# facebookresearch/Active-3D-Vision-and-Touch

Measured on AMD Instinct MI355X. Metric: mesh-recon iters/sec (fwd+bwd, 2562-vert GCN + 10k-pt Chamfer) at bs=64, higher is better.
Workload: dtype f32; 1 GPU; icosphere-4 template (2562 verts, 5120 faces), 3-stage GCN 20x300 cut 0.33, bs=64/GPU, 10000-pt Chamfer x3 draws, Adam, ellipsoid clouds (BASELINE.json configs[1]); global_batch=64, parallelism=dp1

## Files before the change

active-3d-vision-and-touch_amd/csrc/capi.hip:

```cpp
#include <stdarg.h>
#include <stdlib.h>
#include <string.h>

#include "../../include/a3vt.h"
#include <atomic>
#include <mutex>
#include <unordered_map>

#include "common.h"
#include "kernels.h"

namespace a3vt {

static thread_local char g_err[512] = "";

void set_error(const char *fmt, ...) {
  va_list ap;
  va_start(ap, fmt);
  vsnprintf(g_err, sizeof(g_err), fmt, ap);
  va_end(ap);
}

__device__ float g_zero_page[64];
static const float *zero_page() {
// ... 1634 lines not shown
  return launch_conv5_up3(grad_out, batch, out_height, out_width, image, grad_in, static_cast<hipStream_t>(stream));
}

size_t a3vt_conv5_wrw_scratch_bytes(int cin, int cout) {
  return ((cin == 16 || cin == 32) && (cout == 16 || cout == 32)) || (cin == 3 && (cout == 3 || cout == 16)) ? conv5_wrw_scratch_bytes(cin, cout) : 0;
}

int a3vt_conv5_weight_grad(const void *x, const void *grad_out, int batch, int height, int width, int cin, int cout, int stride,
                           float *grad_weight, void *scratch, size_t scratch_bytes, void *stream) {
  A3VT_CHECK_ARG(x && grad_out && grad_weight && scratch);
  A3VT_CHECK_ARG(conv5_shape_ok(cin, cout, stride));
  A3VT_CHECK_ARG(batch > 0 && height >= 3 && width >= 3 && (long long)batch * height * width <= (1ll << 31) / 32);
  A3VT_CHECK_ARG((reinterpret_cast<uintptr_t>(scratch) & 15) == 0);
  A3VT_CHECK_ARG((reinterpret_cast<uintptr_t>(x) & (cin == 3 ? 1 : 15)) == 0 && (reinterpret_cast<uintptr_t>(grad_out) & (cout == 3 ? 1 : 15)) == 0);
  A3VT_CHECK_ARG(scratch_bytes >= conv5_wrw_scratch_bytes(cin, cout));
  ProfScope psc(PROF_ENC, static_cast<hipStream_t>(stream));
  return launch_conv5_wrw(x, grad_out, batch, height, width, cin, cout, stride, grad_weight, scratch, static_cast<hipStream_t>(stream));
}

int a3vt_adam_chunk_elems(void) { return adam_chunk_elems(); }

int a3vt_adam_step(void *const *param, const void *const *grad, void *const *exp_avg, void *const *exp_avg_sq,
                   const long long *numel, const int *chunk_tensor, const long long *chunk_off, int n_chunks, double lr, double beta1,
                   double beta2, double eps, double weight_decay, long long step, void *stream) {
  A3VT_CHECK_ARG(n_chunks >= 0 && step >= 1);
  A3VT_CHECK_ARG(n_chunks == 0 || (param && grad && exp_avg && exp_avg_sq && numel && chunk_tensor && chunk_off));
  A3VT_CHECK_ARG(lr >= 0.0 && beta1 >= 0.0 && beta1 < 1.0 && beta2 >= 0.0 && beta2 < 1.0 && eps >= 0.0 && weight_decay >= 0.0);
  ProfScope psc(PROF_OPT, static_cast<hipStream_t>(stream));
  return launch_adam(param, grad, exp_avg, exp_avg_sq, numel, chunk_tensor, chunk_off, n_chunks, lr, beta1, beta2, eps, weight_decay, step,
                     static_cast<hipStream_t>(stream));
}

int a3vt_adam_step_clamp(void *const *param, void *const *grad, void *const *exp_avg, void *const *exp_avg_sq, const long long *numel,
                         const int *chunk_tensor, const long long *chunk_off, int n_chunks, double lr, double beta1, double beta2,
                         double eps, double weight_decay, long long step, double grad_clamp, void *stream) {
  A3VT_CHECK_ARG(n_chunks >= 0 && step >= 1 && grad_clamp > 0.0);
  A3VT_CHECK_ARG(n_chunks == 0 || (param && grad && exp_avg && exp_avg_sq && numel && chunk_tensor && chunk_off));
  A3VT_CHECK_ARG(lr >= 0.0 && beta1 >= 0.0 && beta1 < 1.0 && beta2 >= 0.0 && beta2 < 1.0 && eps >= 0.0 && weight_decay >= 0.0);
  ProfScope psc(PROF_OPT, static_cast<hipStream_t>(stream));
  return launch_adam(param, const_cast<const void *const *>(grad), exp_avg, exp_avg_sq, numel, chunk_tensor, chunk_off, n_chunks, lr, beta1,
                     beta2, eps, weight_decay, step, static_cast<hipStream_t>(stream), grad_clamp);
}

int a3vt_profile_enable(int on) {
  g_prof.on = on != 0;
  g_prof.used = 0;
  return 0;
}

int a3vt_profile_read_classes(double *total_ms, int *count, int n) {
  A3VT_CHECK_ARG(total_ms && count && n >= 0);
  for (int c = 0; c < n; ++c) { total_ms[c] = 0.0; count[c] = 0; }
  for (int i = 0; i < g_prof.used; ++i) {
    if (hipEventSynchronize(g_prof.ev[i][1]) != hipSuccess) { set_error("profile_read: event sync failed"); return -2; }
    float ms = 0.f;
    if (hipEventElapsedTime(&ms, g_prof.ev[i][0], g_prof.ev[i][1]) != hipSuccess) continue;
    if (g_prof.cls[i] >= n) continue;
    total_ms[g_prof.cls[i]] += ms;
    count[g_prof.cls[i]] += 1;
  }
  g_prof.used = 0;
  return PROF_CLASSES;
}

int a3vt_profile_read(double *total_ms, int *count) {
  const int rc = a3vt_profile_read_classes(total_ms, count, 3);
  return rc < 0 ? rc : 0;
}

int a3vt_dbg_path_counts(long long *counts, int n, int reset) {
  A3VT_CHECK_ARG(n >= 0 && (counts != nullptr || n == 0));
  for (int i = 0; i < n; ++i) counts[i] = i < PATH_COUNT ? g_path_counts[i].load(std::memory_order_relaxed) : 0;
  if (reset)
    for (auto &c : g_path_counts) c.store(0, std::memory_order_relaxed);
  return PATH_COUNT;
}

int a3vt_dbg_csr_algo(int algo) {
  A3VT_CHECK_ARG(algo >= 0 && algo <= 2);
  g_csr_algo = algo;
  return 0;
}

int a3vt_split3_bf16(const float *x, size_t n, uint16_t *hi, uint16_t *mid, uint16_t *lo, void *stream) {
  A3VT_CHECK_ARG(n == 0 || (x && hi && mid && lo));
  return launch_split3(x, n, hi, mid, lo, static_cast<hipStream_t>(stream));
}

int a3vt_check_finite(const float *data, size_t n, int32_t *flag, void *stream) {
  A3VT_CHECK_ARG(data && flag);
  return launch_check_finite(data, n, flag, static_cast<hipStream_t>(stream));
}

}
```

active-3d-vision-and-touch_amd/csrc/gcn_csrq.hip:

```cpp
#include "common.h"
#include "kernels.h"

namespace a3vt {

using f32x4 = __attribute__((ext_vector_type(4))) float;

constexpr int kCsrqThreads = 512;
constexpr int kHeavyDegQ = 64;
constexpr int kEllW = 8;

using i32x2 = __attribute__((ext_vector_type(2))) int;
__device__ __forceinline__ float bits_to_f32(int x) { return __builtin_bit_cast(float, x); }
__device__ __forceinline__ int f32_to_bits(float x) { return __builtin_bit_cast(int, x); }
__global__ void csr_ell_build_kernel(const int32_t *__restrict__ rowptr, const int32_t *__restrict__ colidx,
                                     const float *__restrict__ val, int n_vert, i32x2 *__restrict__ ell,
                                     int32_t *__restrict__ degs) {
  const int v = blockIdx.x * blockDim.x + threadIdx.x;
  if (v >= n_vert) return;
  const int e0 = rowptr[v], n = rowptr[v + 1] - e0;
  degs[v] = n;
#pragma unroll
  for (int j = 0; j < kEllW; ++j)
    ell[(size_t)j * n_vert + v] = j < n ? i32x2{colidx[e0 + j], f32_to_bits(val[e0 + j])} : i32x2{n_vert, 0};
}
size_t csrq_ell_ints(int n_vert) { return (size_t)n_vert * (2 * kEllW + 1) + 64; }
int launch_csrq_ell(const int32_t *rowptr, const int32_t *col, const float *val, int n_vert, int32_t *ell, hipStream_t s) {
  A3VT_LAUNCH(csr_ell_build_kernel, dim3(cdiv(n_vert, 256)), dim3(256), 0, s, rowptr, col, val, n_vert,
              reinterpret_cast<i32x2 *>(ell), ell + (size_t)n_vert * 2 * kEllW);
  A3VT_CHECK_LAUNCH();
  return 0;
}

template <int MODE, int VPT>
__global__ __launch_bounds__(kCsrqThreads) void csrq_kernel(const float *__restrict__ srcq, int nq, int parts,
                                                            const float *__restrict__ bias, int c,
                                                            const int32_t *__restrict__ rowptr,
                                                            const int32_t *__restrict__ colidx,
                                                            const float *__restrict__ val, int n_vert, int batch,
                                                            float *__restrict__ dst, int nq_dst,
                                                            uint8_t *__restrict__ signq, int relu, int heavy_thresh,
                                                            float *__restrict__ db_slab,
                                                            const int32_t *__restrict__ ellbuf) {
  extern __shared__ __attribute__((aligned(16))) float lds_raw[];
  __shared__ float red[2][kCsrqThreads / 64][4];
  const i32x2 *ell = reinterpret_cast<const i32x2 *>(ellbuf);
  const int32_t *degs = ellbuf + (size_t)n_vert * 2 * kEllW;
  f32x4 *tile0 = reinterpret_cast<f32x4 *>(lds_raw);
  const int xcd = blockIdx.x & 7, loc = blockIdx.x >> 3;
  const int jm = loc / parts, part = loc - jm * parts;
  const int b = xcd + 8 * jm;
  if (b >= batch) return;
  const int q_lo = part * nq / parts, q_hi = (part + 1) * nq / parts;
  if (q_lo >= q_hi) return;

  int vv[VPT], dg[VPT];
  bool on[VPT];
  int cj[VPT][kEllW];
  float wj[VPT][kEllW];
#pragma unroll
  for (int k = 0; k < VPT; ++k) {
    const int v = threadIdx.x + k * kCsrqThreads;
    on[k] = v < n_vert;
    vv[k] = on[k] ? v : n_vert - 1;
    dg[k] = degs[vv[k]];
#pragma unroll
    for (int j = 0; j < kEllW; ++j) {
      const i32x2 e = ell[(size_t)j * n_vert + vv[k]];
      const int e0 = e[0], e1 = e[1];
      cj[k][j] = e0;
      wj[k][j] = bits_to_f32(e1);
    }
  }

  auto fetch = [&](int q, int k, f32x4 &v4, unsigned &bits) {
    const size_t plane = ((size_t)b * nq + q) * n_vert;
    v4 = reinterpret_cast<const f32x4 *>(srcq)[plane + vv[k]];
    bits = MODE == 1 ? signq[plane + vv[k]] : 0u;
  };
  auto park = [&](f32x4 *tile, int q, int k, f32x4 v4, unsigned bits) {
    if (MODE == 1) {
#pragma unroll
      for (int t = 0; t < 4; ++t) v4[t] = ((bits >> t) & 1u) ? v4[t] : 0.f;
    }
    (void)q;
    tile[vv[k]] = v4;
  };

  if (threadIdx.x < 2) tile0[(size_t)threadIdx.x * (n_vert + 1) + n_vert] = f32x4{0.f, 0.f, 0.f, 0.f};
  {
    f32x4 v4[VPT];
    unsigned bits[VPT];
#pragma unroll
    for (int k = 0; k < VPT; ++k) fetch(q_lo, k, v4[k], bits[k]);
#pragma unroll
    for (int k = 0; k < VPT; ++k) park(tile0, q_lo, k, v4[k], bits[k]);
  }
  __syncthreads();

  for (int q = q_lo; q < q_hi; ++q) {
    const int par = (q - q_lo) & 1;
    const f32x4 *tile = tile0 + (size_t)par * (n_vert + 1);
    f32x4 *tnext = tile0 + (size_t)(par ^ 1) * (n_vert + 1);
    const int ch = q * 4;
    const size_t plane = ((size_t)b * nq + q) * n_vert;
    const int qn = q + 1 < q_hi ? q + 1 : q;
    f32x4 nv4[VPT];
    unsigned nbits[VPT];
#pragma unroll
    for (int k = 0; k < VPT; ++k) fetch(qn, k, nv4[k], nbits[k]);
    f32x4 bs = {0.f, 0.f, 0.f, 0.f};
    if (MODE == 0) {
#pragma unroll
      for (int t = 0; t < 4; ++t)
        if (ch + t < c) bs[t] = bias[ch + t];
    }
    f32x4 bsum = {0.f, 0.f, 0.f, 0.f};
#pragma unroll
    for (int k = 0; k < VPT; ++k) {
      __builtin_amdgcn_sched_barrier(0);
      const int v = vv[k];
      const f32x4 own = tile[v];
      if (MODE == 1) {
#pragma unroll
        for (int t = 0; t < 4; ++t) bsum[t] += on[k] ? own[t] : 0.f;
      }
      f32x4 acc = {0.f, 0.f, 0.f, 0.f};
#pragma unroll
      for (int j = 0; j < kEllW; ++j) {
        {
          const f32x4 r = tile[cj[k][j]];
          const float w = wj[k][j];
          acc[0] = __builtin_fmaf(w, r[0], acc[0]);
          acc[1] = __builtin_fmaf(w, r[1], acc[1]);
          acc[2] = __builtin_fmaf(w, r[2], acc[2]);
          acc[3] = __builtin_fmaf(w, r[3], acc[3]);
        }
      }
      if (dg[k] > kEllW && dg[k] <= heavy_thresh) {
        const int ea = rowptr[v];
        for (int e = ea + kEllW; e < ea + dg[k]; ++e) {
          const f32x4 r = tile[colidx[e]];
          const float w = val[e];
#pragma unroll
          for (int t = 0; t < 4; ++t) acc[t] = __builtin_fmaf(w, r[t], acc[t]);
        }
      }
      if (!on[k] || dg[k] > heavy_thresh) continue;
      f32x4 o;
      if (MODE == 0) {
        unsigned bits = 0;
#pragma unroll
        for (int t = 0; t < 4; ++t) {
          const float pre = ch + t < c ? acc[t] + bs[t] : own[t];
          o[t] = (pre > 0.f || !relu) ? pre : 0.f;
          bits |= (pre > 0.f ? 1u : 0u) << t;
        }
        if (signq) signq[plane + v] = (uint8_t)bits;
      } else {
#pragma unroll
        for (int t = 0; t < 4; ++t) o[t] = ch + t < c ? acc[t] : own[t];
      }
      *reinterpret_cast<f32x4 *>(dst + ((((size_t)b * nq_dst + q) * n_vert) + v) * 4) = o;
    }
    __builtin_amdgcn_sched_barrier(0);
    if (MODE == 1) {
#pragma unroll
      for (int t = 0; t < 4; ++t) bsum[t] = wave_sum(bsum[t]);
      if ((threadIdx.x & 63) == 0) {
#pragma unroll
        for (int t = 0; t < 4; ++t) red[par][threadIdx.x >> 6][t] = bsum[t];
      }
    }
    if (q + 1 < q_hi) {
#pragma unroll
      for (int k = 0; k < VPT; ++k) park(tnext, q + 1, k, nv4[k], nbits[k]);
    }
    __syncthreads();
    if (MODE == 1 && threadIdx.x < 4) {
      float sacc = 0.f;
#pragma unroll
      for (int w = 0; w < kCsrqThreads / 64; ++w) sacc += red[par][w][threadIdx.x];
      db_slab[(size_t)b * (nq * 4) + ch + threadIdx.x] = sacc;
    }
  }
}

template <int MODE>
__global__ __launch_bounds__(256) void csrq_heavy_kernel(const float *__restrict__ srcq, int nq,
                                                         const float *__restrict__ bias, int c,
                                                         const int32_t *__restrict__ rowptr,
                                                         const int32_t *__restrict__ colidx,
                                                         const float *__restrict__ val, int n_vert, int batch,
                                                         const int32_t *__restrict__ heavy, float *__restrict__ dst,
                                                         int nq_dst, uint8_t *__restrict__ signq, int relu) {
  __shared__ f32x4 red[8][32];
  const int hl = threadIdx.x & 31, sub = threadIdx.x >> 5;
  const int count = heavy[0];
  const bool on = hl < nq;
  const int ch = hl * 4;
  for (long long item = blockIdx.x; item < (long long)count * batch; item += gridDim.x) {
    const int v = heavy[64 + (int)(item % count)];
    const long long b = item / count;
    const size_t plane = ((size_t)b * nq + (on ? hl : 0)) * n_vert;
    const f32x4 *src = reinterpret_cast<const f32x4 *>(srcq) + plane;
    const int e0 = rowptr[v], e1 = rowptr[v + 1];
    const int per = ((e1 - e0 + 7) / 8 + 3) & ~3;
    const int s0 = min(e1, e0 + sub * per), s1 = min(e1, s0 + per);
    f32x4 acc = {0.f, 0.f, 0.f, 0.f};
    if (on) {
      for (int e = s0; e < s1; ++e) {
        const int cc = colidx[e];
        f32x4 r = src[cc];
        if (MODE == 1) {
          const unsigned bits = signq[plane + cc];
#pragma unroll
          for (int t = 0; t < 4; ++t) r[t] = ((bits >> t) & 1u) ? r[t] : 0.f;
        }
#pragma unroll
        for (int t = 0; t < 4; ++t) acc[t] = __builtin_fmaf(val[e], r[t], acc[t]);
      }
    }
    red[sub][hl] = acc;
    __syncthreads();
    if (sub == 0 && on) {
      f32x4 a = red[0][hl];
#pragma unroll
      for (int r = 1; r < 8; ++r) a += red[r][hl];
      f32x4 own = src[v];
      f32x4 o;
      if (MODE == 0) {
        unsigned bits = 0;
#pragma unroll
        for (int t = 0; t < 4; ++t) {
          const float pre = ch + t < c ? a[t] + bias[ch + t] : own[t];
          o[t] = (pre > 0.f || !relu) ? pre : 0.f;
          bits |= (pre > 0.f ? 1u : 0u) << t;
        }
        if (signq) signq[plane + v] = (uint8_t)bits;
      } else {
        const unsigned bits = signq[plane + v];
#pragma unroll
        for (int t = 0; t < 4; ++t) {
          own[t] = ((bits >> t) & 1u) ? own[t] : 0.f;
          o[t] = ch + t < c ? a[t] : own[t];
        }
      }
      *reinterpret_cast<f32x4 *>(dst + ((((size_t)b * nq_dst + hl) * n_vert) + v) * 4) = o;
    }
    __syncthreads();
  }
}

int csrq_max_degree() { return kEllW; }
bool csrq_fits(int n_vert, int cut_len) {
  return cut_len > 0 && pad4(cut_len) <= 128 && n_vert <= 6 * kCsrqThreads && ((size_t)n_vert + 1) * 32 <= 158 * 1024;
}

template <int MODE, int VPT>
static int launch_csrq_vpt(const float *srcq, int nq, const float *bias, int c, const int32_t *rowptr, const int32_t *col,
                           const float *val, const int32_t *heavy, const int32_t *ell, int n_vert, int batch, float *dst,
                           int nq_dst, uint8_t *signq, int relu, float *db_slab, hipStream_t s) {
  const size_t shmem = ((size_t)n_vert + 1) * 32;
  static OncePerDevice once;
  once.run([] {
    (void)hipFuncSetAttribute((const void *)csrq_kernel<MODE, VPT>, hipFuncAttributeMaxDynamicSharedMemorySize, 158 * 1024);
  });
  int parts = 256 / (((batch + 7) / 8) * 8);
  parts = parts < 1 ? 1 : parts > nq ? nq : parts;
  const int grid = 8 * ((batch + 7) / 8) * parts;
  A3VT_LAUNCH((csrq_kernel<MODE, VPT>), dim3(grid), dim3(kCsrqThreads), shmem, s, srcq, nq, parts, bias, c, rowptr, col, val,
              n_vert, batch, dst, nq_dst, signq, relu, heavy ? kHeavyDegQ : 0x7fffffff, db_slab, ell);
  A3VT_CHECK_LAUNCH();
  return 0;
}

template <int MODE>
static int launch_csrq(const float *srcq, const float *bias, int c, const int32_t *rowptr, const int32_t *col,
                       const float *val, const int32_t *heavy, const int32_t *ell, int n_vert, int batch, float *dst,
                       int nq_dst, uint8_t *signq, int relu, float *db_slab, hipStream_t s) {
  const int nq = pad4(c) / 4;
  if (!csrq_fits(n_vert, c) || nq_dst < nq || (MODE == 1 && (!signq || !db_slab))) {
    set_error("csrq: n_vert=%d c=%d output planes=%d unsupported", n_vert, c, nq_dst);
    return -1;
  }
  int rc;
  if (n_vert <= 4 * kCsrqThreads)
    rc = launch_csrq_vpt<MODE, 4>(srcq, nq, bias, c, rowptr, col, val, heavy, ell, n_vert, batch, dst, nq_dst, signq, relu, db_slab, s);
  else
    rc = launch_csrq_vpt<MODE, 6>(srcq, nq, bias, c, rowptr, col, val, heavy, ell, n_vert, batch, dst, nq_dst, signq, relu, db_slab, s);
  if (rc) return rc;
  if (heavy) {
    A3VT_LAUNCH(csrq_heavy_kernel<MODE>, dim3(2048), dim3(256), 0, s, srcq, nq, bias, c, rowptr, col, val, n_vert, batch,
                heavy, dst, nq_dst, signq, relu);
    A3VT_CHECK_LAUNCH();
  }
  return 0;
}

int launch_csrq_fwd(const float *zq, const float *bias, int c, const int32_t *rowptr, const int32_t *col,
                    const float *val, const int32_t *heavy, const int32_t *ell, int n_vert, int batch, float *yq,
                    int yq_quads, uint8_t *signq, int relu, hipStream_t s) {
  return launch_csrq<0>(zq, bias, c, rowptr, col, val, heavy, ell, n_vert, batch, yq, yq_quads, signq, relu, nullptr, s);
}
int launch_csrq_bwd(const float *gq, int c, const int32_t *rowptrT, const int32_t *colT, const float *valT,
                    const int32_t *heavyT, const int32_t *ellT, int n_vert, int batch, float *dzaq,
                    const uint8_t *signq, float *db_slab, hipStream_t s) {
  return launch_csrq<1>(gq, nullptr, c, rowptrT, colT, valT, heavyT, ellT, n_vert, batch, dzaq, pad4(c) / 4,
                        const_cast<uint8_t *>(signq), 0, db_slab, s);
}

}
```

active-3d-vision-and-touch_amd/lib.py:

```python
import ctypes
import os
import subprocess

_HERE = os.path.dirname(os.path.abspath(__file__))
CSRC = os.path.join(_HERE, "csrc")
LIB_PATH = os.environ.get("A3VT_LIB", os.path.join(_HERE, "liba3vt.so"))
SOURCES = ["capi.hip", "gcn_gemm.hip", "gcn_gemmw.hip", "gcn_dww.hip", "gcn_gemm16.hip", "gcn_gemm3.hip", "gcn_csr.hip", "gcn_csrq.hip", "gcn_csrqs.hip", "gcn_bf16s.hip", "posenc.hip", "posenc_wide.hip", "bias_grad.hip", "bnrelu.hip", "conv5.hip", "adam.hip", "sample.hip", "chamfer.hip", "nn_prune.hip",
           "pooling.hip", "fold.hip", "ddqn.hip", "qnet_input.hip"]
EXTRA_FLAGS = {"chamfer.hip": ["-fno-slp-vectorize"], "nn_prune.hip": ["-fno-slp-vectorize"],
               "gcn_csrq.hip": ["-fno-slp-vectorize"], "gcn_csrqs.hip": ["-fno-slp-vectorize"],
               "gcn_gemmw.hip": ["-std=c++20"], "gcn_dww.hip": ["-std=c++20"]}

_vp, _i, _sz, _u64 = ctypes.c_void_p, ctypes.c_int, ctypes.c_size_t, ctypes.c_uint64


class AdjSplit(ctypes.Structure):
    _fields_ = [("rowptr", _vp), ("col", _vp), ("scale", _vp), ("cls", _vp),
                ("max_degree", ctypes.c_int32), ("n_seam", ctypes.c_int32), ("n_centre", ctypes.c_int32)]


SIGNATURES = {
    "a3vt_version": (_i, []),
    "a3vt_last_error": (ctypes.c_char_p, []),
    "a3vt_csr_validate": (_i, [_vp, _vp, _i, _i]),
    "a3vt_gcn_stack_scratch_bytes": (_sz, [_i, _i, _i, _i, _i, _i, _i]),
    "a3vt_gcn_stack_mask_bytes": (_sz, [_i, _i, _i, _i, _i]),
    "a3vt_gcn_stack_scratch_bytes_mode": (_sz, [_i, _i, _i, _i, _i, _i, _i, _i]),
    "a3vt_gcn_stack_stash_bytes": (_i, [_i, _i, _i, _i, _i, _i, _vp, _vp]),
    "a3vt_gcn_stack_fwd": (_i, [_vp, _i, _i, _vp, _vp, _i, _i, _i, _vp, _vp, _vp, _i, _i, _i, _i, _vp, _vp, _vp, _vp, _vp]),
    "a3vt_gcn_stack_bwd": (_i, [_vp, _i, _i, _vp, _vp, _i, _i, _i, _vp, _vp, _vp, _vp, _vp, _vp, _i, _i, _i, _i,
                                _vp, _vp, _vp, _vp, _vp, _vp, _vp, _vp]),
    "a3vt_gcn_stack_bwd_acc": (_i, [_vp, _i, _i, _vp, _vp, _i, _i, _i, _vp, _vp, _vp, _vp, _vp, _vp, _i, _i, _i, _i,
                                    _vp, _vp, _vp, _vp, _vp, _vp, _vp, _i, _vp]),
    "a3vt_adj_split_validate": (_i, [_vp, _vp, _vp, _i, _vp, _vp, _vp, _vp]),
    "a3vt_gcn_stack_fwd_adj": (_i, [_vp, _i, _i, _vp, _vp, _i, _i, _i, _vp, _vp, _vp, _i, _vp, _i, _i, _i, _vp, _vp, _vp, _vp, _vp]),
    "a3vt_gcn_stack_bwd_adj": (_i, [_vp, _i, _i, _vp, _vp, _i, _i, _i, _vp, _vp, _vp, _vp, _vp, _vp, _i, _vp, _i, _i, _i,
                                    _vp, _vp, _vp, _vp, _vp, _vp, _vp, _i, _vp]),
    "a3vt_gcn_layer_scratch_bytes": (_sz, [_i, _i, _i, _i, _i, _i]),
    "a3vt_gcn_layer_fwd": (_i, [_vp, _i, _i, _vp, _vp, _i, _i, _i, _vp, _vp, _vp, _i, _i, _i, _i, _vp, _i, _vp, _vp]),
    "a3vt_gcn_layer_bwd": (_i, [_vp, _i, _i, _vp, _i, _i, _i, _vp, _vp, _vp, _i, _i, _i, _i, _vp, _i, _vp, _i,
                                _vp, _vp, _vp, _vp, _vp]),
    "a3vt_wt_rows": (_i, [_i]),
    "a3vt_wt_ld": (_i, [_i]),
    "a3vt_transpose_weight": (_i, [_vp, _i, _i, _vp, _vp]),
    "a3vt_rowgemm": (_i, [_vp, _i, _i, _i, _vp, _i, _i, _vp, _i, _vp]),
    "a3vt_posenc_param_count": (_sz, [_i]),
    "a3vt_posenc_scratch_bytes": (_sz, [_i, _i]),
    "a3vt_posenc_mask_fwd": (_i, [_vp, _vp, _i, _i, _vp, _vp, _i, _vp]),
    "a3vt_posenc_mask_bwd": (_i, [_vp, _vp, _i, _i, _vp, _vp, _i, _vp, _vp, _vp, _vp]),
    "a3vt_posenc_wide_supported": (_i, [_i]),
    "a3vt_posenc_wide_acts_bytes": (_sz, [_i, _i]),
    "a3vt_posenc_wide_scratch_bytes": (_sz, [_i, _i, _i]),
    "a3vt_posenc_wide_fwd": (_i, [_vp, _vp, _i, _i, _vp, _vp, _i, _vp, _vp, _i, _vp]),
    "a3vt_posenc_wide_bwd": (_i, [_vp, _vp, _i, _i, _vp, _vp, _i, _vp, _vp, _vp, _vp, _i, _vp]),
    "a3vt_image_pool_fwd": (_i, [_vp, _i, _i, _vp, _i, _vp, _vp, _vp, _vp, _vp, _i, _vp]),
    "a3vt_image_pool_fwd_add": (_i, [_vp, _i, _i, _vp, _i, _vp, _vp, _vp, _vp, _vp, _vp, _i, _vp]),
    "a3vt_image_pool_bwd": (_i, [_vp, _i, _i, _vp, _i, _vp, _vp, _vp, _vp, _vp, _i, _vp, _vp, _vp]),
    "a3vt_bias_grad_scratch_bytes": (_sz, [ctypes.c_longlong, _i]),
    "a3vt_bias_grad_nhwc": (_i, [_vp, _i, ctypes.c_longlong, _i, _vp, _vp, _sz, _vp]),
    "a3vt_cast_weights_bf16": (_i, [_i, _vp, _vp, _vp, _vp, _vp, _vp]),
    "a3vt_conv5_supported": (_i, [_i, _i, _i]),
    "a3vt_conv5_image_bytes": (_sz, [_i, _i, _i]),
    "a3vt_conv5_weight_image": (_i, [_vp, _i, _i, _i, _vp, _vp]),
    "a3vt_conv5_nhwc": (_i, [_vp, _i, _i, _i, _i, _i, _i, _i, _vp, _vp, _vp, _vp]),
    "a3vt_conv5_input_grad_3x16s2": (_i, [_vp, _i, _i, _i, _vp, _vp, _vp]),
    "a3vt_conv5_wrw_scratch_bytes": (_sz, [_i, _i]),
    "a3vt_conv5_weight_grad": (_i, [_vp, _vp, _i, _i, _i, _i, _i, _i, _vp, _vp, _sz, _vp]),
    "a3vt_adam_chunk_elems": (_i, []),
    "a3vt_adam_step": (_i, [_vp, _vp, _vp, _vp, _vp, _vp, _vp, _i, ctypes.c_double, ctypes.c_double, ctypes.c_double, ctypes.c_double, ctypes.c_double,
                       ctypes.c_longlong, _vp]),
    "a3vt_adam_step_clamp": (_i, [_vp, _vp, _vp, _vp, _vp, _vp, _vp, _i, ctypes.c_double, ctypes.c_double, ctypes.c_double, ctypes.c_double,
                             ctypes.c_double, ctypes.c_longlong, ctypes.c_double, _vp]),
    "a3vt_bnrelu_scratch_bytes": (_sz, [_i]),
    "a3vt_bnrelu_fwd": (_i, [_vp, ctypes.c_longlong, _i, _vp, _vp, _vp, ctypes.c_float, ctypes.c_float, _vp, _vp, _vp, _vp, _vp, _vp, _sz, _vp]),
    "a3vt_bnrelu_bwd": (_i, [_vp, _vp, ctypes.c_longlong, _i, _vp, _vp, _vp, _vp, _vp, _vp, _sz, _vp]),
    "a3vt_vertex_update": (_i, [_vp, _vp, _i, _i, _i, _vp, _vp]),
    "a3vt_face_cdf": (_i, [_vp, _vp, _i, _i, _i, _vp, _vp]),
    "a3vt_sample_points_fwd": (_i, [_vp, _vp, _vp, _i, _i, _i, _i, _i, _vp, _vp, _vp, _u64, _u64,
                                    _vp, _vp, _vp, _vp, _vp]),
    "a3vt_sample_points_bwd": (_i, [_vp, _i, _i, _i, _i, _i, _vp, _vp, _vp, _vp, _vp, _vp]),
    "a3vt_chamfer_scratch_bytes": (_sz, [_i, _i, _i, _i]),
    "a3vt_chamfer_fwd": (_i, [_vp, _vp, _i, _i, _i, _i, _vp, _vp, _vp, _vp, _vp, _vp, _vp]),
    "a3vt_chamfer_workspace_bytes": (_sz, [_i, _i, _i, _i]),
    "a3vt_chamfer_fwd_ws": (_i, [_vp, _vp, _i, _i, _i, _i, _vp, _vp, _vp, _vp, _vp, _vp, _sz, _i, _vp]),
    "a3vt_chamfer_fwd_shared": (_i, [_vp, _vp, _i, _i, _i, _i, _i, _vp, _vp, _vp, _vp, _vp, _vp, _sz, _i, _vp]),
    "a3vt_chamfer_bwd": (_i, [_vp, _vp, _i, _i, _i, _i, _vp, _vp, _vp, _vp, _vp, _vp]),
    "a3vt_fold_workspace_bytes": (_sz, [_i, _i, _i]),
    "a3vt_fold_fwd": (_i, [_vp, _vp, _i, _vp, _vp, _vp, _vp, _vp, _i, _i, _i, _vp, _vp, _sz, _vp]),
    "a3vt_fold_bwd": (_i, [_vp, _vp, _i, _vp, _vp, _vp, _vp, _vp, _i, _i, _i, _vp, _vp, _vp, _vp, _vp, _vp, _vp, _vp, _sz, _vp]),
    "a3vt_ddqn_td": (_i, [_vp, _vp, _vp, _vp, _vp, _vp, _vp, _i, _i, _i, ctypes.c_float, _vp, _vp, _vp, _vp, _vp]),
    "a3vt_ddqn_td_bwd": (_i, [_vp, _vp, _vp, _i, _i, _vp, _vp]),
    "a3vt_qnet_input_scratch_bytes": (_sz, [_i, _i, _i, _i, _i]),
    "a3vt_qnet_input_fwd": (_i, [_vp, _vp, _vp, _vp, _vp, _vp, _vp, _vp, _vp, _i, _i, _vp, _vp, _vp, _i, _i, _i, _vp, _i, _vp, _vp]),
    "a3vt_qnet_input_bwd": (_i, [_vp, _vp, _vp, _vp, _vp, _vp, _i, _i, _vp, _vp, _vp, _i, _i, _i, _vp, _i, _vp, _i,
                                 _vp, _vp, _vp, _vp, _vp, _vp, _vp, _vp, _vp, _vp]),
    "a3vt_dbg_csr_algo": (_i, [_i]),
    "a3vt_dbg_path_counts": (_i, [_vp, _i, _i]),
    "a3vt_dbg_nn_work": (_i, [_i, _vp]),
    "a3vt_split3_bf16": (_i, [_vp, _sz, _vp, _vp, _vp, _vp]),
    "a3vt_check_finite": (_i, [_vp, _sz, _vp, _vp]),
    "a3vt_profile_enable": (_i, [_i]),
    "a3vt_profile_read": (_i, [_vp, _vp]),
    "a3vt_profile_read_classes": (_i, [_vp, _vp, _i]),
}

_LIB = None


def build(force=False, verbose=False):
    return _build(force, verbose, LIB_PATH, os.path.join(_HERE, "build"))


def _build(force, verbose, lib_path, objdir):
    srcs = [os.path.join(CSRC, s) for s in SOURCES]
    deps = srcs + [os.path.join(CSRC, h) for h in ("common.h", "kernels.h", "gemm_tile.h")] + \
        [os.path.join(_HERE, "..", "include", "a3vt.h")]
    force = force or os.environ.get("A3VT_FORCE_BUILD", "0") not in ("", "0")
    if not force and os.path.exists(lib_path) and all(
            os.path.getmtime(lib_path) >= os.path.getmtime(d) for d in deps if os.path.exists(d)):
        return lib_path
    hipcc = os.environ.get("HIPCC", "/opt/rocm/bin/hipcc")
    if not os.path.exists(hipcc):
        hipcc = "hipcc"
    common = ["-O3", "--offload-arch=gfx950", "-std=c++17", "-fPIC"]
    os.makedirs(objdir, exist_ok=True)
    procs = []
    for name in SOURCES:
        obj = os.path.join(objdir, name.replace(".hip", ".o"))
        cmd = [hipcc, *common, *EXTRA_FLAGS.get(name, []), "-c", os.path.join(CSRC, name), "-o", obj]
        if verbose:
            print(" ".join(cmd))
        procs.append((cmd, subprocess.Popen(cmd), obj))
    objs = []
    for cmd, pr, obj in procs:
        if pr.wait() != 0:
            raise subprocess.CalledProcessError(pr.returncode, cmd)
        objs.append(obj)
    cmd = [hipcc, "--offload-arch=gfx950", "-shared", "-fPIC", *objs, "-o", lib_path]
    if verbose:
        print(" ".join(cmd))
    subprocess.check_call(cmd)
    return lib_path


def load():
    global _LIB
    if _LIB is None:
        if not os.path.exists(LIB_PATH):
            raise RuntimeError(
                f"a3vt: native library {LIB_PATH} is missing. Build it with "
                "`python -c 'import __graft_entry__ as g; g.build()'` (hipcc, gfx950). There is no CPU fallback.")
        import torch
        lib = ctypes.CDLL(LIB_PATH)
        for name, (res, args) in SIGNATURES.items():
            fn = getattr(lib, name)
            fn.restype = res
            fn.argtypes = args
        _LIB = lib
    return _LIB


def check(rc, what):
    if rc != 0:
        msg = load().a3vt_last_error()
        raise RuntimeError(f"a3vt: {what} failed (rc={rc}): {msg.decode() if msg else ''}")


def ptr(t):
    return None if t is None else ctypes.c_void_p(t.data_ptr())
```

include/a3vt.h:

```cpp
#ifndef A3VT_H
#define A3VT_H
#include <stddef.h>
#include <stdint.h>

#ifdef __cplusplus
extern "C" {
#endif

#define A3VT_VERSION 163

int a3vt_version(void);
const char *a3vt_last_error(void);

int a3vt_csr_validate(const int32_t *rowptr_host, const int32_t *col_host, int n_vert, int nnz);

size_t a3vt_gcn_stack_scratch_bytes(int batch, int n_vert, int in_features, int hidden, int num_layers,
                                    int cut_len, int need_backward);
size_t a3vt_gcn_stack_mask_bytes(int batch, int n_vert, int hidden, int num_layers, int cut_len);
size_t a3vt_gcn_stack_scratch_bytes_mode(int batch, int n_vert, int in_features, int hidden, int num_layers,
                                         int cut_len, int need_backward, int gemm_bf16);
int a3vt_gcn_stack_stash_bytes(int batch, int n_vert, int hidden, int num_layers, int cut_len, int gemm_bf16,
                               size_t *acts_bytes, size_t *mask_bytes);

int a3vt_gcn_stack_fwd(const float *feats, int ld_feats, int in_features,
// ... 85 lines not shown
int a3vt_posenc_wide_fwd(const float *verts, const float *mask, int m, int input_size, const float *pe_params,
                         float *feats, int ld_feats, float *acts, float *scratch, int gemm_bf16, void *stream);
int a3vt_posenc_wide_bwd(const float *verts, const float *mask, int m, int input_size, const float *pe_params,
                         const float *grad_feats, int ld_feats, const float *acts, float *grad_verts,
                         float *grad_params, float *scratch, int gemm_bf16, void *stream);

int a3vt_image_pool_fwd(const float *verts, int batch, int n_vert, const float *proj_host, int n_maps,
                        const float *const *maps, const int *chans, const int *heights, const int *widths,
                        float *feats, int ld_feats, void *stream);
int a3vt_image_pool_fwd_add(const float *verts, int batch, int n_vert, const float *proj_host, int n_maps,
                            const float *const *maps, const int *chans, const int *heights, const int *widths,
                            const float *base, float *feats, int ld_feats, void *stream);
int a3vt_image_pool_bwd(const float *verts, int batch, int n_vert, const float *proj_host, int n_maps,
                        const float *const *maps, const int *chans, const int *heights, const int *widths,
                        const float *grad_feats, int ld_feats, float *const *grad_maps, float *grad_verts,
                        void *stream);

size_t a3vt_bias_grad_scratch_bytes(long long rows, int channels);
int a3vt_bias_grad_nhwc(const void *grad, int bf16, long long rows, int channels, float *out, void *scratch,
                        size_t scratch_bytes, void *stream);

size_t a3vt_bnrelu_scratch_bytes(int channels);
int a3vt_bnrelu_fwd(const void *x, long long rows, int channels, const float *gamma, const float *beta, const float *pre_bias,
                    float eps, float momentum, float *running_mean, float *running_var, long long *num_batches_tracked, void *y,
                    float *save, void *scratch, size_t scratch_bytes, void *stream);
int a3vt_bnrelu_bwd(const void *dy, const void *x, long long rows, int channels, const float *save, void *dx, float *dgamma,
                    float *dbeta, float *dx_colsum, void *scratch, size_t scratch_bytes, void *stream);

int a3vt_cast_weights_bf16(int n, const float *const *src, void *const *dst, const long long *outer, const int *inner,
                           const int *hw, void *stream);

int a3vt_conv5_supported(int cin, int cout, int stride);
size_t a3vt_conv5_image_bytes(int cout, int cin, int flip);
int a3vt_conv5_weight_image(const float *weight, int cout, int cin, int flip, void *image, void *stream);
int a3vt_conv5_nhwc(const void *x, int batch, int height, int width, int cin, int cout, int stride, int pad, const void *image,
                    const float *bias, void *y, void *stream);

int a3vt_conv5_input_grad_3x16s2(const void *grad_out, int batch, int out_height, int out_width, const void *image, void *grad_in,
                                 void *stream);

size_t a3vt_conv5_wrw_scratch_bytes(int cin, int cout);
int a3vt_conv5_weight_grad(const void *x, const void *grad_out, int batch, int height, int width, int cin, int cout, int stride,
                           float *grad_weight, void *scratch, size_t scratch_bytes, void *stream);

int a3vt_adam_chunk_elems(void);
int a3vt_adam_step(void *const *param, const void *const *grad, void *const *exp_avg, void *const *exp_avg_sq,
                   const long long *numel, const int *chunk_tensor, const long long *chunk_off, int n_chunks, double lr, double beta1,
                   double beta2, double eps, double weight_decay, long long step, void *stream);
int a3vt_adam_step_clamp(void *const *param, void *const *grad, void *const *exp_avg, void *const *exp_avg_sq, const long long *numel,
                         const int *chunk_tensor, const long long *chunk_off, int n_chunks, double lr, double beta1, double beta2,
                         double eps, double weight_decay, long long step, double grad_clamp, void *stream);

int a3vt_vertex_update(const float *verts_in, const float *update, int batch, int n_vert, int n_vision,
                       float *verts_out, void *stream);

int a3vt_face_cdf(const float *verts, const int32_t *faces, int batch, int n_vert, int n_faces,
                  float *cdf, void *stream);
int a3vt_sample_points_fwd(const float *verts, const int32_t *faces, const float *cdf,
                           int batch, int n_vert, int n_faces, int draws, int num,
                           const int32_t *face_idx_in, const float *u_in, const float *v_in,
                           uint64_t seed, uint64_t offset,
                           float *points, int32_t *face_idx_out, float *u_out, float *v_out, void *stream);
int a3vt_sample_points_bwd(const int32_t *faces, int batch, int n_vert, int n_faces, int draws, int num,
                           const int32_t *face_idx, const float *u, const float *v,
                           const float *grad_points, float *grad_verts, void *stream);

size_t a3vt_chamfer_scratch_bytes(int draws, int batch, int p, int q);
int a3vt_chamfer_fwd(const float *x, const float *y, int draws, int batch, int p, int q,
                     float *dist_xy, int32_t *idx_xy, float *dist_yx, int32_t *idx_yx, float *cd,
                     void *scratch, void *stream);
size_t a3vt_chamfer_workspace_bytes(int draws, int batch, int p, int q);
int a3vt_chamfer_fwd_ws(const float *x, const float *y, int draws, int batch, int p, int q,
                        float *dist_xy, int32_t *idx_xy, float *dist_yx, int32_t *idx_yx, float *cd,
                        void *workspace, size_t workspace_bytes, int algo, void *stream);
int a3vt_chamfer_fwd_shared(const float *x, const float *y, int draws, int batch, int y_batch, int p, int q,
                            float *dist_xy, int32_t *idx_xy, float *dist_yx, int32_t *idx_yx, float *cd,
                            void *workspace, size_t workspace_bytes, int algo, void *stream);
int a3vt_chamfer_bwd(const float *x, const float *y, int draws, int batch, int p, int q,
                     const int32_t *idx_xy, const int32_t *idx_yx, const float *grad_cd,
                     float *grad_x, float *grad_y, void *stream);

int a3vt_dbg_csr_algo(int algo);

int a3vt_dbg_path_counts(long long *counts, int n, int reset);

int a3vt_dbg_nn_work(int enable, unsigned long long *out8);

int a3vt_split3_bf16(const float *x, size_t n, uint16_t *hi, uint16_t *mid, uint16_t *lo, void *stream);

size_t a3vt_fold_workspace_bytes(int batch, int points, int backward);
int a3vt_fold_fwd(const float *bias_s, const float *g, int k, const float *w1g, const float *w2, const float *b2, const float *w3,
                  const float *b3, int batch, int points, int width, float *y, void *workspace, size_t workspace_bytes, void *stream);
int a3vt_fold_bwd(const float *bias_s, const float *g, int k, const float *w1g, const float *w2, const float *b2, const float *w3,
                  const float *dy, int batch, int points, int width, float *d_bias_s, float *dg, float *dw1g, float *dw2, float *db2,
                  float *dw3, float *db3, void *workspace, size_t workspace_bytes, void *stream);

int a3vt_ddqn_td(const float *q_cur, const float *q_next_online, const float *q_next_target, const float *mask, const float *actions,
                 const float *rewards, const float *denom, int batch, int num_actions, int budget, float gamma, float *loss,
                 float *diff, int32_t *best_next, float *target, void *stream);
int a3vt_ddqn_td_bwd(const float *diff, const float *actions, const float *grad_loss, int batch, int num_actions, float *dq_cur,
                     void *stream);

size_t a3vt_qnet_input_scratch_bytes(int batch, int n_vert, int hidden, int cut_len, int backward);
int a3vt_qnet_input_fwd(const float *mesh, const float *w1, const float *b1, const float *w2, const float *b2, const float *comp_s,
                        const float *comp_t, const float *comp_c, const float *bias, int hidden, int cut_len, const int32_t *rowptr,
                        const int32_t *col, const float *val, int max_degree, int n_vert, int batch, float *y, int ld_y,
                        float *scratch, void *stream);
int a3vt_qnet_input_bwd(const float *mesh, const float *w1, const float *b1, const float *w2, const float *b2, const float *comp_c,
                        int hidden, int cut_len, const int32_t *rowptrT, const int32_t *colT, const float *valT, int max_degreeT,
                        int n_vert, int batch, const float *y, int ld_y, const float *grad_y, int ld_gy, float *d_s, float *d_t,
                        float *d_c, float *dw1, float *db1, float *dw2, float *db2, float *grad_bias, float *scratch, void *stream);

int a3vt_check_finite(const float *data, size_t n, int32_t *flag, void *stream);

int a3vt_profile_enable(int on);
int a3vt_profile_read(double *total_ms , int *count );
int a3vt_profile_read_classes(double *total_ms, int *count, int n);

#ifdef __cplusplus
}
#endif
#endif
```

Baseline: 21.94 iters/s.

## Pack ELL columns to 16-bit and peel tail vertices in CSR aggregation kernel

Rebuilds the ELL index image so each vertex's eight neighbour columns are packed as 16-bit pairs in one int4 and its weights sit in two float4s, replacing eight strided int2 loads with three vector loads. The aggregation kernel is re-templated on the number of full 512-vertex slices, with a separately guarded tail slice that whole waves skip. The first feature fetch is also issued before the index loads so the two overlap. Adds a 65535-vertex limit and debug C entry points for testing the aggregation in isolation.

```diff
diff --git a/active-3d-vision-and-touch_amd/csrc/capi.hip b/active-3d-vision-and-touch_amd/csrc/capi.hip
--- a/active-3d-vision-and-touch_amd/csrc/capi.hip
+++ b/active-3d-vision-and-touch_amd/csrc/capi.hip
@@ -1740,6 +1740,54 @@
   return 0;
 }
 
+size_t a3vt_dbg_csr_aggregate_scratch_bytes(int n_vert) {
+  if (n_vert <= 0) return 0;
+  return (align_up(csrq_ell_ints(n_vert), 64) + align_up(csr_heavy_scratch_ints(n_vert), 64)) * sizeof(int32_t);
+}
+
+static int dbg_aggregate_prepare(const int32_t *rowptr, const int32_t *col, const float *val, int n_vert, int max_degree,
+                                 void *scratch, bool sliced, int32_t **ell, int32_t **heavy, hipStream_t s) {
+  *ell = static_cast<int32_t *>(scratch);
+  float *slot = reinterpret_cast<float *>(*ell + align_up(csrq_ell_ints(n_vert), 64));
+  if (int rc = hub_rows(rowptr, n_vert, max_degree, slot, heavy, s)) return rc;
+  return sliced ? launch_csrq_ell(rowptr, col, val, n_vert, *ell, s) : 0;
+}
+
+int a3vt_dbg_csr_aggregate_fwd(const float *z, const float *bias, int c, const int32_t *rowptr, const int32_t *col,
+                               const float *val, int max_degree, int n_vert, int batch, float *y, uint8_t *signs, int relu,
+                               void *scratch, void *stream) {
+  A3VT_CHECK_ARG(z && bias && rowptr && col && val && y && scratch);
+  A3VT_CHECK_ARG(c > 0 && n_vert > 0 && batch > 0);
+  A3VT_CHECK_ARG(reinterpret_cast<uintptr_t>(scratch) % 256 == 0);
+  hipStream_t s = static_cast<hipStream_t>(stream);
+  const bool sliced = g_csr_algo != 1;
+  const int cpad = pad4(c);
+  int32_t *ell, *heavy;
+  if (int rc = dbg_aggregate_prepare(rowptr, col, val, n_vert, max_degree, scratch, sliced, &ell, &heavy, s)) return rc;
+  if (sliced) return launch_csrq_fwd(z, bias, c, rowptr, col, val, heavy, ell, n_vert, batch, y, cpad / 4, signs, relu, s);
+  return launch_csr_fwd(z, cpad, bias, c, rowptr, col, val, heavy, n_vert, batch, y, cpad, signs, cpad / 4, relu, s);
+}
+
+int a3vt_dbg_csr_aggregate_bwd(const float *g, int c, const int32_t *rowptr_t, const int32_t *col_t, const float *val_t,
+                               int max_degree, int n_vert, int batch, float *dza, const uint8_t *signs, float *db_slab,
+                               void *scratch, void *stream) {
+  A3VT_CHECK_ARG(g && rowptr_t && col_t && val_t && dza && db_slab && scratch);
+  A3VT_CHECK_ARG(c > 0 && n_vert > 0 && batch > 0);
+  A3VT_CHECK_ARG(reinterpret_cast<uintptr_t>(scratch) % 256 == 0);
+  hipStream_t s = static_cast<hipStream_t>(stream);
+  const bool sliced = g_csr_algo != 1;
+  A3VT_CHECK_ARG(!sliced || signs);
+  int32_t *ell, *heavy;
+  if (int rc = dbg_aggregate_prepare(rowptr_t, col_t, val_t, n_vert, max_degree, scratch, sliced, &ell, &heavy, s)) return rc;
+  if (sliced) return launch_csrq_bwd(g, c, rowptr_t, col_t, val_t, heavy, ell, n_vert, batch, dza, signs, db_slab, s);
+  return launch_csr_bwd(g, pad4(c), c, rowptr_t, col_t, val_t, heavy, n_vert, batch, dza, pad4(c), db_slab, s);
+}
+
+int a3vt_dbg_csr_aggregate_slabs(int batch, int n_vert) {
+  A3VT_CHECK_ARG(batch > 0 && n_vert > 0);
+  return g_csr_algo != 1 ? batch : csr_bwd_num_slabs(batch, n_vert);
+}
+
 int a3vt_split3_bf16(const float *x, size_t n, uint16_t *hi, uint16_t *mid, uint16_t *lo, void *stream) {
   A3VT_CHECK_ARG(n == 0 || (x && hi && mid && lo));
   return launch_split3(x, n, hi, mid, lo, static_cast<hipStream_t>(stream));
diff --git a/active-3d-vision-and-touch_amd/csrc/gcn_csrq.hip b/active-3d-vision-and-touch_amd/csrc/gcn_csrq.hip
--- a/active-3d-vision-and-touch_amd/csrc/gcn_csrq.hip
+++ b/active-3d-vision-and-touch_amd/csrc/gcn_csrq.hip
@@ -9,29 +9,39 @@
 constexpr int kHeavyDegQ = 64;
 constexpr int kEllW = 8;
 
-using i32x2 = __attribute__((ext_vector_type(2))) int;
-__device__ __forceinline__ float bits_to_f32(int x) { return __builtin_bit_cast(float, x); }
-__device__ __forceinline__ int f32_to_bits(float x) { return __builtin_bit_cast(int, x); }
+using i32x4 = __attribute__((ext_vector_type(4))) int;
 __global__ void csr_ell_build_kernel(const int32_t *__restrict__ rowptr, const int32_t *__restrict__ colidx,
-                                     const float *__restrict__ val, int n_vert, i32x2 *__restrict__ ell,
-                                     int32_t *__restrict__ degs) {
+                                     const float *__restrict__ val, int n_vert, i32x4 *__restrict__ cols,
+                                     f32x4 *__restrict__ wlo, f32x4 *__restrict__ whi, int32_t *__restrict__ degs) {
   const int v = blockIdx.x * blockDim.x + threadIdx.x;
   if (v >= n_vert) return;
   const int e0 = rowptr[v], n = rowptr[v + 1] - e0;
   degs[v] = n;
-#pragma unroll
-  for (int j = 0; j < kEllW; ++j)
-    ell[(size_t)j * n_vert + v] = j < n ? i32x2{colidx[e0 + j], f32_to_bits(val[e0 + j])} : i32x2{n_vert, 0};
-}
-size_t csrq_ell_ints(int n_vert) { return (size_t)n_vert * (2 * kEllW + 1) + 64; }
+  unsigned cc[kEllW];
+  float ww[kEllW];
+#pragma unroll
+  for (int j = 0; j < kEllW; ++j) {
+    cc[j] = j < n ? (unsigned)colidx[e0 + j] : (unsigned)n_vert;
+    ww[j] = j < n ? val[e0 + j] : 0.f;
+  }
+  cols[v] = i32x4{(int)(cc[0] | (cc[1] << 16)), (int)(cc[2] | (cc[3] << 16)), (int)(cc[4] | (cc[5] << 16)), (int)(cc[6] | (cc[7] << 16))};
+  wlo[v] = f32x4{ww[0], ww[1], ww[2], ww[3]};
+  whi[v] = f32x4{ww[4], ww[5], ww[6], ww[7]};
+}
+size_t csrq_ell_ints(int n_vert) { return (size_t)n_vert * (3 * 4 + 1) + 64; }
 int launch_csrq_ell(const int32_t *rowptr, const int32_t *col, const float *val, int n_vert, int32_t *ell, hipStream_t s) {
+  if (n_vert <= 0 || n_vert >= 65535) {
+    set_error("csrq index image: n_vert=%d does not fit 16-bit columns", n_vert);
+    return -1;
+  }
   A3VT_LAUNCH(csr_ell_build_kernel, dim3(cdiv(n_vert, 256)), dim3(256), 0, s, rowptr, col, val, n_vert,
-              reinterpret_cast<i32x2 *>(ell), ell + (size_t)n_vert * 2 * kEllW);
+              reinterpret_cast<i32x4 *>(ell), reinterpret_cast<f32x4 *>(ell + (size_t)n_vert * 4),
+              reinterpret_cast<f32x4 *>(ell + (size_t)n_vert * 8), ell + (size_t)n_vert * 12);
   A3VT_CHECK_LAUNCH();
   return 0;
 }
 
-template <int MODE, int VPT>
+template <int MODE, int NF>
 __global__ __launch_bounds__(kCsrqThreads) void csrq_kernel(const float *__restrict__ srcq, int nq, int parts,
                                                             const float *__restrict__ bias, int c,
                                                             const int32_t *__restrict__ rowptr,
@@ -41,10 +51,13 @@
                                                             uint8_t *__restrict__ signq, int relu, int heavy_thresh,
                                                             float *__restrict__ db_slab,
                                                             const int32_t *__restrict__ ellbuf) {
+  constexpr int VPT = NF + 1;
   extern __shared__ __attribute__((aligned(16))) float lds_raw[];
   __shared__ float red[2][kCsrqThreads / 64][4];
-  const i32x2 *ell = reinterpret_cast<const i32x2 *>(ellbuf);
-  const int32_t *degs = ellbuf + (size_t)n_vert * 2 * kEllW;
+  const i32x4 *ecols = reinterpret_cast<const i32x4 *>(ellbuf);
+  const f32x4 *ewlo = reinterpret_cast<const f32x4 *>(ellbuf + (size_t)n_vert * 4);
+  const f32x4 *ewhi = reinterpret_cast<const f32x4 *>(ellbuf + (size_t)n_vert * 8);
+  const int32_t *degs = ellbuf + (size_t)n_vert * 12;
   f32x4 *tile0 = reinterpret_cast<f32x4 *>(lds_raw);
   const int xcd = blockIdx.x & 7, loc = blockIdx.x >> 3;
   const int jm = loc / parts, part = loc - jm * parts;
@@ -53,48 +66,57 @@
   const int q_lo = part * nq / parts, q_hi = (part + 1) * nq / parts;
   if (q_lo >= q_hi) return;
 
-  int vv[VPT], dg[VPT];
-  bool on[VPT];
-  int cj[VPT][kEllW];
-  float wj[VPT][kEllW];
-#pragma unroll
-  for (int k = 0; k < VPT; ++k) {
-    const int v = threadIdx.x + k * kCsrqThreads;
-    on[k] = v < n_vert;
-    vv[k] = on[k] ? v : n_vert - 1;
-    dg[k] = degs[vv[k]];
-#pragma unroll
-    for (int j = 0; j < kEllW; ++j) {
-      const i32x2 e = ell[(size_t)j * n_vert + vv[k]];
-      const int e0 = e[0], e1 = e[1];
-      cj[k][j] = e0;
-      wj[k][j] = bits_to_f32(e1);
-    }
-  }
+  const int wave = __builtin_amdgcn_readfirstlane((int)(threadIdx.x >> 6));
+  const bool tail = NF * kCsrqThreads + wave * 64 < n_vert;
+  const bool on_tail = NF * kCsrqThreads + (int)threadIdx.x < n_vert;
+  int vv[VPT];
+#pragma unroll
+  for (int k = 0; k < NF; ++k) vv[k] = threadIdx.x + k * kCsrqThreads;
+  vv[NF] = on_tail ? NF * kCsrqThreads + (int)threadIdx.x : n_vert - 1;
 
   auto fetch = [&](int q, int k, f32x4 &v4, unsigned &bits) {
     const size_t plane = ((size_t)b * nq + q) * n_vert;
     v4 = reinterpret_cast<const f32x4 *>(srcq)[plane + vv[k]];
     bits = MODE == 1 ? signq[plane + vv[k]] : 0u;
   };
-  auto park = [&](f32x4 *tile, int q, int k, f32x4 v4, unsigned bits) {
+  auto park = [&](f32x4 *tile, int k, f32x4 v4, unsigned bits) {
     if (MODE == 1) {
 #pragma unroll
       for (int t = 0; t < 4; ++t) v4[t] = ((bits >> t) & 1u) ? v4[t] : 0.f;
     }
-    (void)q;
     tile[vv[k]] = v4;
   };
 
+  f32x4 fv4[VPT];
+  unsigned fbits[VPT];
+#pragma unroll
+  for (int k = 0; k < NF; ++k) fetch(q_lo, k, fv4[k], fbits[k]);
+  if (tail) fetch(q_lo, NF, fv4[NF], fbits[NF]);
+
+  int dg[VPT];
+  int cj[VPT][kEllW];
+  float wj[VPT][kEllW];
+  auto entries = [&](int k) {
+    dg[k] = degs[vv[k]];
+    const i32x4 cp = ecols[vv[k]];
+    const f32x4 w0 = ewlo[vv[k]], w1 = ewhi[vv[k]];
+#pragma unroll
+    for (int p = 0; p < 4; ++p) {
+      const int word = cp[p];
+      cj[k][2 * p] = word & 0xffff;
+      cj[k][2 * p + 1] = (int)((unsigned)word >> 16);
+      wj[k][p] = w0[p];
+      wj[k][4 + p] = w1[p];
+    }
+  };
+#pragma unroll
+  for (int k = 0; k < NF; ++k) entries(k);
+  if (tail) entries(NF);
+
   if (threadIdx.x < 2) tile0[(size_t)threadIdx.x * (n_vert + 1) + n_vert] = f32x4{0.f, 0.f, 0.f, 0.f};
-  {
-    f32x4 v4[VPT];
-    unsigned bits[VPT];
-#pragma unroll
-    for (int k = 0; k < VPT; ++k) fetch(q_lo, k, v4[k], bits[k]);
-#pragma unroll
-    for (int k = 0; k < VPT; ++k) park(tile0, q_lo, k, v4[k], bits[k]);
-  }
+#pragma unroll
+  for (int k = 0; k < NF; ++k) park(tile0, k, fv4[k], fbits[k]);
+  if (tail) park(tile0, NF, fv4[NF], fbits[NF]);
   __syncthreads();
 
   for (int q = q_lo; q < q_hi; ++q) {
@@ -107,7 +129,8 @@
     f32x4 nv4[VPT];
     unsigned nbits[VPT];
 #pragma unroll
-    for (int k = 0; k < VPT; ++k) fetch(qn, k, nv4[k], nbits[k]);
+    for (int k = 0; k < NF; ++k) fetch(qn, k, nv4[k], nbits[k]);
+    if (tail) fetch(qn, NF, nv4[NF], nbits[NF]);
     f32x4 bs = {0.f, 0.f, 0.f, 0.f};
     if (MODE == 0) {
 #pragma unroll
@@ -115,14 +138,12 @@
         if (ch + t < c) bs[t] = bias[ch + t];
     }
     f32x4 bsum = {0.f, 0.f, 0.f, 0.f};
-#pragma unroll
-    for (int k = 0; k < VPT; ++k) {
-      __builtin_amdgcn_sched_barrier(0);
+    auto vertex = [&](int k, bool on) {
       const int v = vv[k];
       const f32x4 own = tile[v];
       if (MODE == 1) {
 #pragma unroll
-        for (int t = 0; t < 4; ++t) bsum[t] += on[k] ? own[t] : 0.f;
+        for (int t = 0; t < 4; ++t) bsum[t] += on ? own[t] : 0.f;
       }
       f32x4 acc = {0.f, 0.f, 0.f, 0.f};
 #pragma unroll
@@ -145,7 +166,7 @@
           for (int t = 0; t < 4; ++t) acc[t] = __builtin_fmaf(w, r[t], acc[t]);
         }
       }
-      if (!on[k] || dg[k] > heavy_thresh) continue;
+      if (!on || dg[k] > heavy_thresh) return;
       f32x4 o;
       if (MODE == 0) {
         unsigned bits = 0;
@@ -161,7 +182,14 @@
         for (int t = 0; t < 4; ++t) o[t] = ch + t < c ? acc[t] : own[t];
       }
       *reinterpret_cast<f32x4 *>(dst + ((((size_t)b * nq_dst + q) * n_vert) + v) * 4) = o;
-    }
+    };
+#pragma unroll
+    for (int k = 0; k < NF; ++k) {
+      __builtin_amdgcn_sched_barrier(0);
+      vertex(k, true);
+    }
+    __builtin_amdgcn_sched_barrier(0);
+    if (tail) vertex(NF, on_tail);
     __builtin_amdgcn_sched_barrier(0);
     if (MODE == 1) {
 #pragma unroll
@@ -173,7 +201,8 @@
     }
     if (q + 1 < q_hi) {
 #pragma unroll
-      for (int k = 0; k < VPT; ++k) park(tnext, q + 1, k, nv4[k], nbits[k]);
+      for (int k = 0; k < NF; ++k) park(tnext, k, nv4[k], nbits[k]);
+      if (tail) park(tnext, NF, nv4[NF], nbits[NF]);
     }
     __syncthreads();
     if (MODE == 1 && threadIdx.x < 4) {
@@ -256,19 +285,19 @@
   return cut_len > 0 && pad4(cut_len) <= 128 && n_vert <= 6 * kCsrqThreads && ((size_t)n_vert + 1) * 32 <= 158 * 1024;
 }
 
-template <int MODE, int VPT>
-static int launch_csrq_vpt(const float *srcq, int nq, const float *bias, int c, const int32_t *rowptr, const int32_t *col,
+template <int MODE, int NF>
+static int launch_csrq_nf(const float *srcq, int nq, const float *bias, int c, const int32_t *rowptr, const int32_t *col,
                            const float *val, const int32_t *heavy, const int32_t *ell, int n_vert, int batch, float *dst,
                            int nq_dst, uint8_t *signq, int relu, float *db_slab, hipStream_t s) {
   const size_t shmem = ((size_t)n_vert + 1) * 32;
   static OncePerDevice once;
   once.run([] {
-    (void)hipFuncSetAttribute((const void *)csrq_kernel<MODE, VPT>, hipFuncAttributeMaxDynamicSharedMemorySize, 158 * 1024);
+    (void)hipFuncSetAttribute((const void *)csrq_kernel<MODE, NF>, hipFuncAttributeMaxDynamicSharedMemorySize, 158 * 1024);
   });
   int parts = 256 / (((batch + 7) / 8) * 8);
   parts = parts < 1 ? 1 : parts > nq ? nq : parts;
   const int grid = 8 * ((batch + 7) / 8) * parts;
-  A3VT_LAUNCH((csrq_kernel<MODE, VPT>), dim3(grid), dim3(kCsrqThreads), shmem, s, srcq, nq, parts, bias, c, rowptr, col, val,
+  A3VT_LAUNCH((csrq_kernel<MODE, NF>), dim3(grid), dim3(kCsrqThreads), shmem, s, srcq, nq, parts, bias, c, rowptr, col, val,
               n_vert, batch, dst, nq_dst, signq, relu, heavy ? kHeavyDegQ : 0x7fffffff, db_slab, ell);
   A3VT_CHECK_LAUNCH();
   return 0;
@@ -284,10 +313,18 @@
     return -1;
   }
   int rc;
-  if (n_vert <= 4 * kCsrqThreads)
-    rc = launch_csrq_vpt<MODE, 4>(srcq, nq, bias, c, rowptr, col, val, heavy, ell, n_vert, batch, dst, nq_dst, signq, relu, db_slab, s);
-  else
-    rc = launch_csrq_vpt<MODE, 6>(srcq, nq, bias, c, rowptr, col, val, heavy, ell, n_vert, batch, dst, nq_dst, signq, relu, db_slab, s);
+#define A3VT_CSRQ_NF(nf)                                                                                                  \
+  case nf:                                                                                                                \
+    rc = launch_csrq_nf<MODE, nf>(srcq, nq, bias, c, rowptr, col, val, heavy, ell, n_vert, batch, dst, nq_dst, signq, relu, \
+                                  db_slab, s);                                                                            \
+    break;
+  switch ((n_vert - 1) / kCsrqThreads) {
+    A3VT_CSRQ_NF(0) A3VT_CSRQ_NF(1) A3VT_CSRQ_NF(2) A3VT_CSRQ_NF(3) A3VT_CSRQ_NF(4) A3VT_CSRQ_NF(5)
+    default:
+      set_error("csrq: n_vert=%d unsupported", n_vert);
+      return -1;
+  }
+#undef A3VT_CSRQ_NF
   if (rc) return rc;
   if (heavy) {
     A3VT_LAUNCH(csrq_heavy_kernel<MODE>, dim3(2048), dim3(256), 0, s, srcq, nq, bias, c, rowptr, col, val, n_vert, batch,
diff --git a/active-3d-vision-and-touch_amd/lib.py b/active-3d-vision-and-touch_amd/lib.py
--- a/active-3d-vision-and-touch_amd/lib.py
+++ b/active-3d-vision-and-touch_amd/lib.py
@@ -96,6 +96,10 @@
                                  _vp, _vp, _vp, _vp, _vp, _vp, _vp, _vp, _vp, _vp]),
     "a3vt_dbg_csr_algo": (_i, [_i]),
     "a3vt_dbg_path_counts": (_i, [_vp, _i, _i]),
+    "a3vt_dbg_csr_aggregate_scratch_bytes": (_sz, [_i]),
+    "a3vt_dbg_csr_aggregate_slabs": (_i, [_i, _i]),
+    "a3vt_dbg_csr_aggregate_fwd": (_i, [_vp, _vp, _i, _vp, _vp, _vp, _i, _i, _i, _vp, _vp, _i, _vp, _vp]),
+    "a3vt_dbg_csr_aggregate_bwd": (_i, [_vp, _i, _vp, _vp, _vp, _i, _i, _i, _vp, _vp, _vp, _vp, _vp]),
     "a3vt_dbg_nn_work": (_i, [_i, _vp]),
     "a3vt_split3_bf16": (_i, [_vp, _sz, _vp, _vp, _vp, _vp]),
     "a3vt_check_finite": (_i, [_vp, _sz, _vp, _vp]),
diff --git a/include/a3vt.h b/include/a3vt.h
--- a/include/a3vt.h
+++ b/include/a3vt.h
@@ -191,6 +191,15 @@
 
 int a3vt_dbg_csr_algo(int algo);
 
+size_t a3vt_dbg_csr_aggregate_scratch_bytes(int n_vert);
+int a3vt_dbg_csr_aggregate_slabs(int batch, int n_vert);
+int a3vt_dbg_csr_aggregate_fwd(const float *z, const float *bias, int c, const int32_t *rowptr, const int32_t *col,
+                               const float *val, int max_degree, int n_vert, int batch, float *y, uint8_t *signs, int relu,
+                               void *scratch, void *stream);
+int a3vt_dbg_csr_aggregate_bwd(const float *g, int c, const int32_t *rowptr_t, const int32_t *col_t, const float *val_t,
+                               int max_degree, int n_vert, int batch, float *dza, const uint8_t *signs, float *db_slab,
+                               void *scratch, void *stream);
+
 int a3vt_dbg_path_counts(long long *counts, int n, int reset);
 
 int a3vt_dbg_nn_work(int enable, unsigned long long *out8);
```

Result: no change. 22.11 iters/s, median of 6 (+0.8%).
